# Jingliang-Duan/DSAC-v2

Hardware: NVIDIA H100
Metric: DSAC-T gradient-steps/sec @ batch 4096 (Humanoid-dim) (higher is better)
Workload: dtype bf16x3

## Files before the change

### dsac-v2_b200/_lib.py

```python
from __future__ import annotations

import ctypes as C
import os

_HERE = os.path.dirname(os.path.abspath(__file__))
LIB_PATH = os.environ.get("DSACT_LIB") or os.path.join(_HERE, "libdsact.so")

ABI_VERSION = 4
MAX_HIDDEN = 6
NUM_STATS = 16

ACTIVATIONS = {"linear": 0, "relu": 1, "gelu": 2, "tanh": 3, "sigmoid": 4, "elu": 5, "selu": 6}
GEMM_MODES = {"fp32": 0, "bf16x3": 1, "bf16": 2}
ACT_DISTS = {"TanhGaussDistribution": 0, "GaussDistribution": 1}
POLICY_STDS = {"mlp_shared": 0, "mlp_separated": 1, "parameter": 2}

STATE_STDSUM = 4
STATE_ACC = 16
STATE_STATS = 48


class Config(C.Structure):
    _fields_ = [
        ("abi_version", C.c_int32), ("obs_dim", C.c_int32), ("act_dim", C.c_int32),
# ... 110 lines not shown
    "dsact_seed": (C.c_int, [C.c_void_p, C.c_uint64]),
    "dsact_set_carry": (C.c_int, [C.c_void_p, C.c_float, C.c_float, C.c_int64, C.c_int64, C.c_void_p]),
    "dsact_step": (C.c_int, [C.c_void_p, C.POINTER(Batch), C.POINTER(Noise), C.c_int64, C.c_void_p]),
    "dsact_step_host": (C.c_int, [C.c_void_p, C.POINTER(Batch), C.POINTER(Noise), C.c_int64, C.c_void_p]),
    "dsact_stage_host": (C.c_int, [C.c_void_p, C.POINTER(Batch), C.POINTER(Batch), C.c_void_p]),
    "dsact_stage_release": (C.c_int, [C.c_void_p, C.c_void_p]),
    "dsact_grad_phase1": (C.c_int, [C.c_void_p, C.POINTER(Batch), C.POINTER(Noise), C.c_void_p]),
    "dsact_grad_phase2": (C.c_int, [C.c_void_p, C.c_int64, C.c_void_p]),
    "dsact_compute_grads": (C.c_int, [C.c_void_p, C.POINTER(Batch), C.POINTER(Noise), C.c_void_p]),
    "dsact_apply": (C.c_int, [C.c_void_p, C.c_int64, C.c_void_p]),
    "dsact_read_stats": (C.c_int, [C.c_void_p, C.c_int64, C.c_void_p, C.c_void_p]),
    "dsact_replay_bind": (C.c_int, [C.c_void_p, C.POINTER(Replay)]),
    "dsact_replay_add": (C.c_int, [C.c_void_p] + [C.c_void_p] * 6 + [C.c_int64, C.c_int64, C.c_void_p]),
    "dsact_replay_sample": (C.c_int, [C.c_void_p, C.c_int32, C.c_int64, C.c_void_p, C.POINTER(Batch), C.c_void_p]),
    "dsact_replay_step": (C.c_int, [C.c_void_p, C.c_int32, C.c_int64, C.c_void_p, C.POINTER(Noise), C.c_int64, C.c_void_p]),
    "dsact_replay_steps": (C.c_int, [C.c_void_p, C.c_int32, C.c_int32, C.c_int64, C.c_void_p, C.POINTER(Noise), C.c_void_p,
                                     C.c_int64, C.c_void_p]),
    "dsact_dp_export": (C.c_int, [C.c_void_p, C.c_void_p, C.POINTER(C.c_int64)]),
    "dsact_dp_connect": (C.c_int, [C.c_void_p, C.c_int32, C.c_int32, C.c_void_p]),
    "dsact_dp_step": (C.c_int, [C.c_void_p, C.POINTER(Batch), C.POINTER(Noise), C.c_int64, C.c_int64, C.c_void_p]),
    "dsact_dp_replay_step": (C.c_int, [C.c_void_p, C.c_int32, C.c_int64, C.c_void_p, C.POINTER(Noise), C.c_int64, C.c_int64,
                                       C.c_void_p]),
    "dsact_v1_query_layout": (C.c_int, [C.POINTER(Config), C.POINTER(V1Options), C.POINTER(Layout)]),
    "dsact_v1_create": (C.c_int, [C.POINTER(Config), C.POINTER(V1Options), C.c_int, C.POINTER(C.c_void_p)]),
    "dsact_cnn_query_layout": (C.c_int, [C.POINTER(CnnConfig), C.POINTER(Layout)]),
    "dsact_cnn_create": (C.c_int, [C.POINTER(CnnConfig), C.c_int, C.POINTER(C.c_void_p)]),
    "dsact_profile_step": (C.c_int, [C.c_void_p, C.POINTER(Batch), C.POINTER(Noise), C.c_int64, C.c_void_p, C.POINTER(Profile)]),
    "dsact_launch_count": (C.c_int64, [C.c_void_p]),
    "dsact_last_call_launches": (C.c_int32, [C.c_void_p]),
    "dsact_cnn_test_conv": (C.c_int, [C.c_int32] * 8 + [C.c_void_p] * 7 + [C.c_int32] * 4 + [C.c_void_p]),
    "dsact_test_gemm": (C.c_int, [C.c_void_p, C.c_int32, C.POINTER(TestLayer), C.c_int32, C.c_int32, C.c_void_p]),
    "dsact_test_chain": (C.c_int, [C.c_void_p, C.c_int32, C.c_int32, C.POINTER(C.c_int32), C.c_int32, C.c_int32, C.c_int32,
                                   C.c_int32, C.c_void_p, C.POINTER(TestChainPass), C.c_int32, C.c_void_p]),
    "dsact_test_rows": (C.c_int, [C.c_void_p, C.POINTER(TestRowIo), C.c_void_p]),
    "dsact_test_apply": (C.c_int, [C.c_void_p, C.c_int32, C.c_int32, C.c_int32, C.c_int32, C.c_int64, C.c_int32, C.c_void_p]),
    "dsact_test_dp_attach": (C.c_int, [C.c_void_p, C.c_int32, C.c_int32, C.POINTER(C.c_void_p), C.POINTER(C.c_void_p),
                                       C.POINTER(C.c_int64)]),
    "dsact_test_dp": (C.c_int, [C.c_void_p, C.c_int32, C.POINTER(TestDpIo), C.c_void_p]),
}

_lib = None


class DsactError(RuntimeError):
    pass


def load() -> C.CDLL:
    global _lib
    if _lib is not None:
        return _lib
    if not os.path.exists(LIB_PATH):
        raise DsactError(
            f"{LIB_PATH} is missing: build it with `python -c 'import __graft_entry__ as g; g.build()'` "
            "(nvcc, sm_90a). There is no CPU fallback for the DSAC-T update path.")
    lib = C.CDLL(LIB_PATH)
    for name, (res, args) in SYMBOLS.items():
        fn = getattr(lib, name)
        fn.restype = res
        fn.argtypes = args
    if lib.dsact_abi_version() != ABI_VERSION:
        raise DsactError(f"libdsact.so ABI {lib.dsact_abi_version()} != binding ABI {ABI_VERSION}")
    _lib = lib
    return lib


# ... 4 lines not shown
```

### dsac-v2_b200/csrc/engine.cu

```cuda
#include <cuda_runtime.h>
#include <stdarg.h>
#include <stdio.h>
#include <stdlib.h>
#include <string.h>

#include <algorithm>
#include <cmath>

#include <vector>

#include "../../include/dsact.h"
#include "gemm_simt.cuh"
#include "kernels.cuh"
#include "tc_host.cuh"
#include "chain_tc.cuh"
#include "wgrad_tc.cuh"
#include "dp_peer.cuh"

using namespace dsact;

static thread_local char g_err[512] = "";
static int fail(int code, const char* fmt, ...) {
  va_list ap;
  va_start(ap, fmt);
  vsnprintf(g_err, sizeof(g_err), fmt, ap);
  va_end(ap);
  return code;
}
#define CUDA_TRY(x)                                                                       \
  do {                                                                                    \
    cudaError_t e_ = (x);                                                                 \
    if (e_ != cudaSuccess) return fail(DSACT_ECUDA, "%s failed: %s", #x, cudaGetErrorString(e_)); \
  } while (0)

struct Net {
  int L;
  int s[DSACT_MAX_HIDDEN + 2];
  int64_t w[DSACT_MAX_HIDDEN + 1], b[DSACT_MAX_HIDDEN + 1], n;
  void build(int in, const int32_t* hidden, int L_, int out) {
    L = L_;
    s[0] = in;
    for (int j = 0; j < L; ++j) s[j + 1] = hidden[j];
    s[L + 1] = out;
    n = 0;
    for (int j = 0; j <= L; ++j) {
      w[j] = n; n += (int64_t)s[j + 1] * s[j];
      b[j] = n; n += s[j + 1];
    }
// ... 543 lines not shown
      int blocks = (int)((total + 255) / 256);
      if (blocks < 1) blocks = 1;
      if (blocks > 2 * h->num_sms) blocks = 2 * h->num_sms;
      grid += blocks;
    }
    if (pro) {
      pro->img_blocks = grid;
      launch_k(step_prologue_kernel, grid + pro->zero_blocks + pro->noise_blocks, 256, 0, c, g, *pro);
    } else {
      launch_k(image_kernel, grid, 256, 0, c, g);
    }
    c.done();
    g.n = 0;
  }
};

static ImgOut img_out(const MlpHandle* h, const ImgSlot& s) {
  ImgOut o;
  o.p = nullptr; o.pitch = 0; o.planes = h->passes() == 3 ? 2 : 1; o.plane = 0;
  if (h->tc() && s.off >= 0) { o.p = reinterpret_cast<__nv_bfloat16*>(h->W() + s.off); o.pitch = s.pitch; o.plane = s.plane; }
  return o;
}
static ImgOut img_out_of(const MlpHandle* h, const Img& i) {
  ImgOut o;
  o.p = i.p; o.pitch = i.p ? i.pitch : 0; o.planes = h->passes() == 3 ? 2 : 1; o.plane = i.p ? i.plane : 0;
  return o;
}


struct ChainBuild {
  ChainGroup g;
  int grid = 0, stage_b = 16 * 128;
  int b_mn = -1;
  double flops = 0.0;
  bool ok = true;
  explicit ChainBuild(int passes) { memset(&g, 0, sizeof(g)); g.passes = passes; }
  ChainPass& begin(const Img& a0, const Img& a1, int M) {
    ChainPass& P = g.p[g.n++];
    P.n_layers = 0; P.M = M; P.tile_start = grid;
    grid += (M + TC_BM - 1) / TC_BM;
    ok = ok && make_map(&P.mapA[0], a0, TC_BM);
    if (a1.p) ok = ok && make_map(&P.mapA[1], a1, TC_BM);
    return P;
  }
  ChainLayer& layer(ChainPass& P, const Img& wimg, bool b_mn, int N, int K0, int K1, int kB1) {
    ChainLayer& L = P.L[P.n_layers++];
    L.N = N; L.ldc = N; L.bn = (N + 15) / 16 * 16;
    const int o = b_mn ? 1 : 0;
    if (this->b_mn >= 0 && this->b_mn != o) ok = false;
    this->b_mn = o;
    L.kblocks[0] = (K0 + TC_BK - 1) / TC_BK; L.kblocks[1] = (K1 + TC_BK - 1) / TC_BK;
    L.kB0[0] = 0; L.kB0[1] = kB1;
    ok = ok && make_map(&L.mapB, wimg, b_mn ? 64 : L.bn);
    const int sb = (L.bn + 63) / 64 * 8192;
    if (sb > stage_b) stage_b = sb;
    flops += 2.0 * P.M * N * ((double)K0 + K1);
    return L;
  }
  void image(ChainLayer& L, Img im) {
    if (!im.p) return;
    im.width = (L.N + 7) / 8 * 8;
    L.img = 1;
    ok = ok && make_map(&L.mapImg, im, TC_BM);
  }
};

static void launch_chain(MlpHandle* h, ChainBuild& cb, int cls, Ctx& c) {
  if (cb.g.n == 0) return;
  for (int i = 0; i < cb.g.n; ++i)
    for (int j = 0; j < cb.g.p[i].n_layers; ++j)
      if (cb.g.p[i].L[j].ldc != cb.g.p[i].L[j].N && cb.g.p[i].L[j].Zout) cb.ok = false;
  if (!cb.ok) { c.err = cudaErrorInvalidValue; return; }
  static unsigned long long* dbg = nullptr;
  const bool debug = getenv("DSACT_TC_DEBUG") != nullptr;
  if (debug && !dbg) cudaMalloc(&dbg, sizeof(unsigned long long) * TC_DBG_SLOTS * 4096);
  if (debug && cb.grid <= 4096) { cudaMemsetAsync(dbg, 0, sizeof(unsigned long long) * TC_DBG_SLOTS * cb.grid, c.s); cb.g.dbg = dbg; }
  const int planes = cb.g.passes == 3 ? 2 : 1;
  const int stages = planes == 2 ? 2 : 4;
  const int smem = chain_smem_bytes(stages, planes, cb.stage_b);
  if (!h->chain_attr_done) {
    cudaFuncSetAttribute(tc_chain_kernel<true, false>, cudaFuncAttributeMaxDynamicSharedMemorySize, 227 * 1024);
    cudaFuncSetAttribute(tc_chain_kernel<true, true>, cudaFuncAttributeMaxDynamicSharedMemorySize, 227 * 1024);
    cudaFuncSetAttribute(tc_chain_kernel<false, false>, cudaFuncAttributeMaxDynamicSharedMemorySize, 227 * 1024);
    cudaFuncSetAttribute(tc_chain_kernel<false, true>, cudaFuncAttributeMaxDynamicSharedMemorySize, 227 * 1024);
    h->chain_attr_done = true;
  }
  if (planes == 2) {
    if (cb.b_mn) launch_k(tc_chain_kernel<true, true>, cb.grid, CH_THREADS, smem, c, cb.g, stages, cb.stage_b);
    else launch_k(tc_chain_kernel<true, false>, cb.grid, CH_THREADS, smem, c, cb.g, stages, cb.stage_b);
  } else {
    if (cb.b_mn) launch_k(tc_chain_kernel<false, true>, cb.grid, CH_THREADS, smem, c, cb.g, stages, cb.stage_b);
    else launch_k(tc_chain_kernel<false, false>, cb.grid, CH_THREADS, smem, c, cb.g, stages, cb.stage_b);
  }
  c.done(cls, cb.flops);
  c.check();
  if (debug && cb.g.dbg) {
    cudaStreamSynchronize(c.s);
    std::vector<unsigned long long> hbuf(TC_DBG_SLOTS * (size_t)cb.grid);
    cudaMemcpy(hbuf.data(), dbg, sizeof(unsigned long long) * TC_DBG_SLOTS * cb.grid, cudaMemcpyDeviceToHost);
    unsigned long long tmin = ~0ull, tmax = 0;
    for (int i = 0; i < cb.grid; ++i) {
      const unsigned long long* d = &hbuf[TC_DBG_SLOTS * (size_t)i];
      if (d[0] < tmin) tmin = d[0];
      if (d[6] > tmax) tmax = d[6];
    }
    fprintf(stderr, "[chain_debug] class %d passes %d grid %d span %.1f us\n", cls, cb.g.n, cb.grid, (tmax - tmin) / 1000.0);
    for (int pi = 0; pi < cb.g.n; ++pi) {
      const unsigned long long* d = &hbuf[TC_DBG_SLOTS * (size_t)cb.g.p[pi].tile_start];
      fprintf(stderr, "  pass %d: setup %.1f first-load %.1f |", pi, (d[1] - d[0]) / 1e3, (d[2] - d[0]) / 1e3);
      for (int j = 0; j < cb.g.p[pi].n_layers; ++j)
        fprintf(stderr, " L%d mma-done %.1f epilogue %.1f operand %.1f |", j, (d[8 + 3 * j] - d[0]) / 1e3, (d[9 + 3 * j] - d[0]) / 1e3,
                (d[10 + 3 * j] - d[0]) / 1e3);
      fprintf(stderr, " end %.1f\n", (d[6] - d[0]) / 1e3);
    }
  }
}

struct ChainIo {
  Img w[DSACT_MAX_HIDDEN + 1];
  float* z[DSACT_MAX_HIDDEN] = {};
  Img img[DSACT_MAX_HIDDEN];
  float* colsum[DSACT_MAX_HIDDEN] = {};
};

static ChainPass& chain_fwd_layers(ChainBuild& cb, const Net& net, const float* Wbase, const ChainIo& io, const Img& in0, int k0,
                                   const Img& in1, int k1, int kB1, int B, int act, float* out, int out_ld = 0) {
  ChainPass& P = cb.begin(in0, in1, B);
  for (int j = 0; j <= net.L; ++j) {
    ChainLayer& L = j == 0 ? cb.layer(P, io.w[0], false, net.s[1], k0, k1, kB1) : cb.layer(P, io.w[j], false, net.s[j + 1], net.s[j], 0, 0);
    const bool last = j == net.L;
    L.epi = last ? EPI_STORE : EPI_BIAS_ACT;
    L.act = act;
    L.bias = Wbase + net.b[j];
    if (last) { L.C = out; if (out_ld) L.ldc = out_ld; }
    else {
      L.Zout = io.z[j];
      cb.image(L, io.img[j]);
    }
  }
  return P;
}

static ChainPass& chain_dgrad_layers(ChainBuild& cb, const Net& net, const ChainIo& io, const Img& dout, int B, int act,
                                     float* dact_out, int act_col_img, int act_cols) {
  const Img none;
  ChainPass& P = cb.begin(dout, none, B);
// ... 1634 lines not shown
        x.b = mem.img(t.K0, t.N);
        ibt.add(t.B, t.ldb, x.b, t.K0, t.N);
      }
      if (t.img) {
        x.out.p = static_cast<__nv_bfloat16*>(t.img); x.out.rows = t.M; x.out.width = t.N;
        x.out.pitch = t.img_pitch; x.out.plane = t.img_plane;
      }
      G.wg_off[i] = slab_floats;
      if (variant == V_WGRAD) slab_floats += ((long long)t.M * t.N + 3) / 4 * 4;
    }
    G.push(p, x);
  }
  const int nslabs = 4;
  if (tc) {
    ibt.launch(h, c);
    if (variant == V_WGRAD) {
      G.wg_slab = static_cast<float*>(mem.get(sizeof(float) * (size_t)nslabs * slab_floats));
      G.wg_stride = slab_floats; G.wg_nslabs = nslabs;
      if (G.wg_slab) c.err = cudaMemsetAsync(G.wg_slab, 0xff, sizeof(float) * (size_t)nslabs * slab_floats, c.s);
    }
  }
  if (mem.err == cudaSuccess) launch_group(h, G, variant, c, max_ctas);
  if (tc && variant == V_WGRAD && c.err == cudaSuccess && mem.err == cudaSuccess) {
    for (int i = 0; i < n; ++i) {
      grad_reduce_kernel<<<64, 256, 0, c.s>>>(probs[i].C, G.wg_slab + G.wg_off[i], (long long)probs[i].M * probs[i].N, nslabs,
                                               G.wg_stride);
      c.done();
    }
    c.check();
  }
  return finish_hook(h, c, mem);
}

int dsact_test_chain(dsact_handle* hh, int32_t dgrad, int32_t L, const int32_t* sizes, int32_t K0, int32_t K1, int32_t kB1,
                     int32_t act, const float* params, const dsact_test_chain_pass* passes, int32_t n_passes, void* stream) {
  if (!hh) return fail(DSACT_EINVAL, "null handle");
  int rc = check_mlp(hh, "dsact_test_chain");
  if (rc) return rc;
  MlpHandle* h = mlp(hh);
  if (!h->tc()) return fail(DSACT_EINVAL, "dsact_test_chain: the layer-chain kernel runs in the tensor-core modes only");
  if (!sizes || !params || !passes || L < 0 || L > DSACT_MAX_HIDDEN || n_passes < 1 || n_passes > CH_MAX_PASSES ||
      act < 0 || act > ACT_SELU || (dgrad != 0 && dgrad != 1) || (dgrad && L < 1))
    return fail(DSACT_EINVAL, "bad argument");
  for (int j = 0; j <= L + 1; ++j)
    if (sizes[j] < 1 || (j > 0 && sizes[j] > 256) || (j > 0 && j <= L && sizes[j] % 8))
      return fail(DSACT_EINVAL, "sizes[%d] = %d: widths are >= 1, layer outputs <= 256, hidden widths multiples of 8", j, sizes[j]);
  if (K0 < 1 || K1 < 0 || K0 + K1 != sizes[0] || (K1 > 0 && (kB1 < K0 || kB1 % 8)))
    return fail(DSACT_EINVAL, "layer-0 segments: K0 + K1 == sizes[0], kB1 >= K0, kB1 %% 8 == 0");
  for (int i = 0; i < n_passes; ++i) {
    const dsact_test_chain_pass& q = passes[i];
    if (q.M < 1 || !q.x0 || (!dgrad && (!q.out || (K1 > 0 && !q.x1))) || (dgrad && q.out && K1 == 0) ||
        (q.out_ld != 0 && (dgrad || q.out_ld < sizes[L + 1])))
      return fail(DSACT_EINVAL, "pass %d: bad argument", i);
    for (int j = 0; j < L && dgrad; ++j)
      if (!q.Zin[j]) return fail(DSACT_EINVAL, "pass %d: Zin[%d] is null", i, j);
  }
  CUDA_TRY(cudaSetDevice(h->device));
  Ctx c{(cudaStream_t)stream, 0, cudaSuccess};
  HookScratch mem;
  ImgBatch ibt;
  Net net;
  net.build(sizes[0], sizes + 1, L, sizes[L + 1]);
  ChainIo io;
  for (int j = 0; j <= L; ++j) {
    io.w[j] = mem.img(sizes[j + 1], j == 0 && K1 > 0 ? kB1 + K1 : sizes[j]);
    ibt.reserve(h, c, 1);
    if (j == 0) ibt.add(params + net.w[0], sizes[0], io.w[0], sizes[1], K0, K1, kB1);
    else ibt.add(params + net.w[j], sizes[j], io.w[j], sizes[j + 1], sizes[j]);
  }
  ChainBuild cb(h->passes());
  for (int i = 0; i < n_passes; ++i) {
    const dsact_test_chain_pass& q = passes[i];
    ChainIo pio = io;
    for (int j = 0; j < L; ++j) {
      pio.z[j] = dgrad ? const_cast<float*>(q.Zin[j]) : q.Zout[j];
      pio.colsum[j] = dgrad ? q.colsum[j] : nullptr;
      if (q.img[j]) {
        Img& o = pio.img[j];
        o.p = static_cast<__nv_bfloat16*>(q.img[j]); o.rows = q.M; o.width = sizes[j + 1];
        o.pitch = (sizes[j + 1] + 7) / 8 * 8; o.plane = (long long)o.pitch * q.M;
      }
    }
    const int w0 = dgrad ? sizes[L + 1] : K0;
    ibt.reserve(h, c, 2);
    const Img in0 = mem.img(q.M, w0);
    ibt.add(q.x0, w0, in0, q.M, w0);
    if (dgrad) {
      chain_dgrad_layers(cb, net, pio, in0, q.M, act, q.out, kB1, K1);
    } else {
      Img in1;
      if (K1 > 0) { in1 = mem.img(q.M, K1); ibt.add(q.x1, K1, in1, q.M, K1); }
      chain_fwd_layers(cb, net, params, pio, in0, K0, in1, K1, kB1, q.M, act, q.out, q.out_ld);
    }
  }
  if (mem.err == cudaSuccess) {
    ibt.launch(h, c);
    launch_chain(h, cb, dgrad ? CLS_GEMM_DGRAD : CLS_GEMM_FWD, c);
  }
  return finish_hook(h, c, mem);
}

static int sync_hook(dsact_handle* h, Ctx& c) {
  const cudaError_t e = cudaStreamSynchronize(c.s);
  const cudaError_t err = c.err != cudaSuccess ? c.err : e;
  if (err != cudaSuccess) return fail(DSACT_ECUDA, "launch failed: %s", cudaGetErrorString(err));
  h->launches += c.launches;
  return DSACT_OK;
}

int dsact_test_rows(dsact_handle* h, const dsact_test_row_io* t, void* stream) {
  if (!h || !h->bound) return fail(DSACT_ESTATE, "not bound");
  if (!t) return fail(DSACT_EINVAL, "null rows");
  if (t->kernel < DSACT_TEST_SAMPLE || t->kernel > DSACT_TEST_STATS) return fail(DSACT_EINVAL, "unknown kernel %d", t->kernel);
  const int B = t->batch;
  if (t->kernel != DSACT_TEST_STATS && (B < 1 || B > h->max_batch)) return fail(DSACT_EINVAL, "batch %d outside [1, max_batch]", B);
  if (t->global_batch < (t->kernel == DSACT_TEST_STATS ? 1 : B)) return fail(DSACT_EINVAL, "global_batch < batch");
  if (t->max_blocks < 0) return fail(DSACT_EINVAL, "max_blocks < 0");
  const bool v1 = h->v1, mlp_eng = h->engine == ENGINE_MLP;
  const bool tc = mlp_eng && mlp(h)->tc();
  const int A = h->act_dim, nq = v1 ? 1 : 2;
  const void* imgs[8] = {t->img_act[0], t->img_act[1], t->img_q[0], t->img_q[1], t->img_qa[0], t->img_qa[1], t->img_dlogits,
                         t->img_dlogits_ls};
  for (const void* p : imgs)
    if (p && !tc) return fail(DSACT_EINVAL, "images need a tensor-core mode of the MLP engine");
  auto need = [&](const void* p, const char* what) { return p ? DSACT_OK : fail(DSACT_EINVAL, "%s is null", what); };
  int rc = DSACT_OK;
  RowIo io;
  memset(&io, 0, sizeof(io));
  auto img = [&](void* p, int width) {
    if (!p) return NO_IMG;
    ImgOut o;
    o.p = static_cast<__nv_bfloat16*>(p); o.pitch = (width + 7) / 8 * 8; o.planes = mlp(h)->passes() == 3 ? 2 : 1;
// ... 168 lines not shown
```

### dsac-v2_b200/engine.py

```python
from __future__ import annotations

import ctypes as C
from typing import Dict, Optional, Sequence

import torch

from . import _lib
from ._lib import Batch, Buffers, Config, Layout, Noise, Replay, V1Options, check

STAT_KEYS = [
    "DSAC2/critic_avg_q1-RL iter",
    "DSAC2/critic_avg_q2-RL iter",
    "DSAC2/critic_avg_std1-RL iter",
    "DSAC2/critic_avg_std2-RL iter",
    "DSAC2/critic_avg_min_std1-RL iter",
    "DSAC2/critic_avg_min_std2-RL iter",
    "Loss/Actor loss-RL iter",
    "Loss/Critic loss-RL iter",
    "DSAC2/policy_mean-RL iter",
    "DSAC2/policy_std-RL iter",
    "DSAC2/entropy-RL iter",
    "DSAC2/alpha-RL iter",
    "DSAC2/mean_std1",
    "DSAC2/mean_std2",
# ... 451 lines not shown
        out = {"log_alpha": host[n].clone()}
        for key, tkey, off, cnt, shape in schema:
            out[key] = host[off:off + cnt].view(shape).clone()
            if not grads:
                out[tkey] = thost[off:off + cnt].view(shape).clone()
        return out

    def launch_count(self) -> int:
        return int(self.lib.dsact_launch_count(self.h))

    def last_call_launches(self) -> int:
        return int(self.lib.dsact_last_call_launches(self.h))

    def test_gemm(self, variant: int, A: torch.Tensor, B: torch.Tensor, bias: Optional[torch.Tensor], C_out: torch.Tensor,
                  M: int, N: int, K: int):
        self.test_layers(variant, [dict(M=M, N=N, K0=K, A0=A, B=B, bias=bias, C=C_out)])

    def test_layers(self, variant: int, probs, max_ctas: int = 0):
        arr = (_lib.TestLayer * len(probs))()
        for t, p in zip(arr, probs):
            for k, v in p.items():
                if k == "img":
                    t.img, t.img_pitch, t.img_plane = v.data_ptr(), v.stride(1), v.stride(0)
                elif isinstance(v, torch.Tensor):
                    setattr(t, k, v.data_ptr())
                    ld = {"A0": "lda0", "A1": "lda1", "B": "ldb", "Zin": "ldz", "C": "ldc"}.get(k)
                    if ld and ld not in p:
                        setattr(t, ld, v.stride(0))
                elif v is not None:
                    setattr(t, k, v)
        with torch.cuda.device(self.device):
            check(self.lib.dsact_test_gemm(self.h, variant, arr, len(probs), max_ctas, self._stream()))

    def test_chain(self, dgrad: bool, sizes, K0: int, K1: int, kB1: int, act: int, params: torch.Tensor, passes):
        arr = (_lib.TestChainPass * len(passes))()
        for t, p in zip(arr, passes):
            t.M = p["M"]
            for k in ("x0", "x1", "out"):
                setattr(t, k, _ptr(p.get(k)))
            t.out_ld = int(p.get("out_ld", 0))
            for k in ("Zout", "Zin", "img", "colsum"):
                for j, v in enumerate(p.get(k) or []):
                    getattr(t, k)[j] = _ptr(v)
        sz = (C.c_int32 * len(sizes))(*sizes)
        with torch.cuda.device(self.device):
            check(self.lib.dsact_test_chain(self.h, int(dgrad), len(sizes) - 2, sz, K0, K1, kB1, act, params.data_ptr(), arr,
                                            len(passes), self._stream()))

    def test_rows(self, kernel: str, batch: int, global_batch: Optional[int] = None, max_blocks: int = 0,
                  advance_rng: bool = False, **arrays):
        t = _lib.TestRowIo()
        t.kernel, t.batch = _lib.TEST_KERNELS[kernel], int(batch)
        t.global_batch = int(batch if global_batch is None else global_batch)
        t.max_blocks, t.advance_rng = int(max_blocks), int(bool(advance_rng))
        for k, v in arrays.items():
            if isinstance(v, (list, tuple)):
                for i, x in enumerate(v):
                    getattr(t, k)[i] = _ptr(x)
            else:
                setattr(t, k, v if isinstance(v, int) else _ptr(v))
        with torch.cuda.device(self.device):
            check(self.lib.dsact_test_rows(self.h, C.byref(t), self._stream()))

    def test_apply(self, part: int = 0, fold_slabs: int = 0, scalars_ready: int = 0, tail_rows: int = 0,
                   global_batch: int = 1, max_blocks: int = 0):
        with torch.cuda.device(self.device):
            check(self.lib.dsact_test_apply(self.h, int(part), int(fold_slabs), int(scalars_ready), int(tail_rows),
                                            int(global_batch), int(max_blocks), self._stream()))

    def test_dp_attach(self, rank: int, peers: Sequence["Engine"]) -> torch.Tensor:
        arr = (C.c_void_p * len(peers))(*(p.h.value for p in peers))
        buf, n = C.c_void_p(), C.c_int64()
        with torch.cuda.device(self.device):
            check(self.lib.dsact_test_dp_attach(self.h, int(rank), len(peers), arr, C.byref(buf), C.byref(n)))
        self.dp_world = len(peers)
        self._dp_peers = list(peers)
        return _device_view(buf.value, int(n.value), self.device)

    def test_dp(self, op: str, kind: int = 0, grads: Optional[torch.Tensor] = None, slabs: Optional[torch.Tensor] = None,
                nslabs: int = 0, slab_stride: int = 0, n: int = 0, tail_rows: int = 0, global_batch: int = 1):
# ... 15 lines not shown
```

### include/dsact.h

```cpp
#ifndef DSACT_H
#define DSACT_H

#include <stdint.h>

#ifdef __cplusplus
extern "C" {
#endif

#define DSACT_ABI_VERSION 4
#define DSACT_MAX_HIDDEN 6
#define DSACT_NUM_STATS 16

enum {
  DSACT_OK = 0,
  DSACT_EINVAL = -1,
  DSACT_ECUDA = -2,
  DSACT_ESTATE = -3,
  DSACT_EARCH = -4
};

enum {
  DSACT_ACT_LINEAR = 0, DSACT_ACT_RELU = 1, DSACT_ACT_GELU = 2, DSACT_ACT_TANH = 3,
  DSACT_ACT_SIGMOID = 4, DSACT_ACT_ELU = 5, DSACT_ACT_SELU = 6
};
// ... 156 lines not shown
int dsact_profile_step(dsact_handle *h, const dsact_batch *batch, const dsact_noise *noise, int64_t iteration,
                       void *stream, dsact_profile *out);

typedef struct dsact_test_layer {
  int32_t M, N, K0, K1, kB1;
  const float *A0, *A1, *B;
  int32_t lda0, lda1, ldb;
  int32_t epi, act;
  const float *bias;
  float *Zout;
  const float *Zin;
  int32_t ldz;
  float *colsum;
  float *C;
  int32_t ldc;
  void *img;
  int32_t img_pitch;
  int64_t img_plane;
} dsact_test_layer;
int dsact_test_gemm(dsact_handle *h, int32_t variant, const dsact_test_layer *probs, int32_t n, int32_t max_ctas, void *stream);

typedef struct dsact_test_chain_pass {
  int32_t M;
  const float *x0, *x1;
  float *Zout[DSACT_MAX_HIDDEN];
  const float *Zin[DSACT_MAX_HIDDEN];
  void *img[DSACT_MAX_HIDDEN];
  float *colsum[DSACT_MAX_HIDDEN];
  float *out;
  int32_t out_ld;
} dsact_test_chain_pass;
int dsact_test_chain(dsact_handle *h, int32_t dgrad, int32_t L, const int32_t *sizes, int32_t K0, int32_t K1, int32_t kB1,
                     int32_t act, const float *params, const dsact_test_chain_pass *passes, int32_t n_passes, void *stream);

enum { DSACT_TEST_SAMPLE = 0, DSACT_TEST_LOSS = 1, DSACT_TEST_POLICY_GRAD = 2, DSACT_TEST_STATS = 3 };
typedef struct dsact_test_row_io {
  int32_t kernel, batch;
  int64_t global_batch;
  int32_t max_blocks, advance_rng;
  const float *logits[2], *eps[2];
  float *act[2], *logp[2];
  const float *rew, *done, *z3, *z4;
  const float *out_q[6];
  float *d_out_q[2], *d_out_qa[2];
  const float *d_act[2];
  float *d_logits;
  float *gbias_q[2], *gbias_q_raw[2], *gbias_pi, *gbias_ls;
  void *img_act[2], *img_q[2], *img_qa[2], *img_dlogits;
  float *stats_out;
  void *img_dlogits_ls;
  int32_t split_dlogits;
} dsact_test_row_io;
int dsact_test_rows(dsact_handle *h, const dsact_test_row_io *rows, void *stream);

int dsact_test_apply(dsact_handle *h, int32_t part, int32_t fold_slabs, int32_t scalars_ready, int32_t tail_rows,
                     int64_t global_batch, int32_t max_blocks, void *stream);

int dsact_test_dp_attach(dsact_handle *h, int32_t rank, int32_t world, dsact_handle *const *peers, void **buffer,
                         int64_t *floats);
enum { DSACT_TEST_DP_EXCHANGE = 0, DSACT_TEST_DP_FOLD = 1, DSACT_TEST_DP_REDUCE_SCATTER = 2, DSACT_TEST_DP_APPLY = 3 };
typedef struct dsact_test_dp_io {
  int32_t kind;
  dsact_handle *const *ranks;
  const float *grads, *slabs;
  int32_t nslabs;
  int64_t slab_stride, n;
// ... 21 lines not shown
```

Measured before the change: 2305.

## Add ping-pong two-warpgroup chain kernel selected when grid exceeds one wave

Adds a new fused MLP-chain kernel where each CTA owns two row tiles processed by two consumer warpgroups that alternate tensor-core use through named barriers. One warpgroup's epilogue overlaps the other's WGMMA mainloop, and the weight tiles are split into 128-column halves. The launcher picks this ping-pong variant automatically when the column-split grid would exceed one wave of resident CTAs. The price is a more complex synchronisation scheme, re-created tensor maps, and two half-width B loads per k-block for layers wider than 128.

```diff
diff --git a/dsac-v2_b200/_lib.py b/dsac-v2_b200/_lib.py
--- a/dsac-v2_b200/_lib.py
+++ b/dsac-v2_b200/_lib.py
@@ -166,6 +166,9 @@
     "dsact_test_gemm": (C.c_int, [C.c_void_p, C.c_int32, C.POINTER(TestLayer), C.c_int32, C.c_int32, C.c_void_p]),
     "dsact_test_chain": (C.c_int, [C.c_void_p, C.c_int32, C.c_int32, C.POINTER(C.c_int32), C.c_int32, C.c_int32, C.c_int32,
                                    C.c_int32, C.c_void_p, C.POINTER(TestChainPass), C.c_int32, C.c_void_p]),
+    "dsact_test_chain_tiling": (C.c_int, [C.c_void_p, C.c_int32, C.c_int32, C.c_int32, C.POINTER(C.c_int32), C.c_int32,
+                                          C.c_int32, C.c_int32, C.c_int32, C.c_void_p, C.POINTER(TestChainPass), C.c_int32,
+                                          C.c_void_p]),
     "dsact_test_rows": (C.c_int, [C.c_void_p, C.POINTER(TestRowIo), C.c_void_p]),
     "dsact_test_apply": (C.c_int, [C.c_void_p, C.c_int32, C.c_int32, C.c_int32, C.c_int32, C.c_int64, C.c_int32, C.c_void_p]),
     "dsact_test_dp_attach": (C.c_int, [C.c_void_p, C.c_int32, C.c_int32, C.POINTER(C.c_void_p), C.POINTER(C.c_void_p),
diff --git a/dsac-v2_b200/csrc/chain_pp.cuh b/dsac-v2_b200/csrc/chain_pp.cuh
--- /dev/null
+++ b/dsac-v2_b200/csrc/chain_pp.cuh
@@ -0,0 +1,299 @@
+#pragma once
+#include "chain_tc.cuh"
+
+namespace dsact {
+
+constexpr int PP_HALF = 128;
+constexpr int PP_STAGE_B = PP_HALF * 128;
+constexpr int PP_THREADS = CH_THREADS;
+
+inline int pp_smem_bytes(int stages, int planes) {
+  return stages * planes * PP_STAGE_B + 2 * planes * CH_OPND_PLANE + CH_SCRATCH + 2 * stages * 8 + 1024;
+}
+
+__device__ __forceinline__ uint32_t pp_tid() {
+  uint32_t t;
+  asm volatile("mov.u32 %0, %%tid.x;" : "=r"(t));
+  return t;
+}
+__device__ __forceinline__ int pp_wg() { return (int)(pp_tid() / TC_MMA_THREADS); }
+__device__ __forceinline__ bool pp_lead() { return (pp_tid() & (TC_MMA_THREADS - 1)) == 0; }
+__device__ __forceinline__ void pp_bar() { asm volatile("bar.sync %0, %1;" ::"r"(2 + pp_wg()), "n"(TC_MMA_THREADS) : "memory"); }
+__device__ __forceinline__ void pp_wait_turn() {
+  asm volatile("bar.sync %0, %1;" ::"r"(4 + pp_wg()), "n"(2 * TC_MMA_THREADS) : "memory");
+}
+__device__ __forceinline__ void pp_give_turn() {
+  asm volatile("bar.arrive %0, %1;" ::"r"(5 - pp_wg()), "n"(2 * TC_MMA_THREADS) : "memory");
+}
+
+template <int TB>
+__device__ __forceinline__ void wgmma_n64_hi(float (&d)[128], uint64_t a, uint64_t b) {
+  asm volatile(
+      "{\n\t.reg .pred p;\n\tsetp.ne.b32 p, 1, 0;\n\t"
+      "wgmma.mma_async.sync.aligned.m64n64k16.f32.bf16.bf16 {%0, %1, %2, %3, %4, %5, %6, %7, %8, %9, %10, %11, %12, %13, %14, %15, %16, %17, %18, %19, %20, %21, %22, %23, %24, %25, %26, %27, %28, %29, %30, %31}, %32, %33, p, 1, 1, 0, %34;\n\t}"
+      : "+f"(d[64]), "+f"(d[65]), "+f"(d[66]), "+f"(d[67]), "+f"(d[68]), "+f"(d[69]), "+f"(d[70]), "+f"(d[71]), "+f"(d[72]), "+f"(d[73]), "+f"(d[74]), "+f"(d[75]), "+f"(d[76]), "+f"(d[77]), "+f"(d[78]), "+f"(d[79]), "+f"(d[80]), "+f"(d[81]), "+f"(d[82]), "+f"(d[83]), "+f"(d[84]), "+f"(d[85]), "+f"(d[86]), "+f"(d[87]), "+f"(d[88]), "+f"(d[89]), "+f"(d[90]), "+f"(d[91]), "+f"(d[92]), "+f"(d[93]), "+f"(d[94]), "+f"(d[95])
+      : "l"(a), "l"(b), "n"(TB));
+}
+
+template <int TB>
+__device__ __forceinline__ void wgmma_n128_hi(float (&d)[128], uint64_t a, uint64_t b) {
+  asm volatile(
+      "{\n\t.reg .pred p;\n\tsetp.ne.b32 p, 1, 0;\n\t"
+      "wgmma.mma_async.sync.aligned.m64n128k16.f32.bf16.bf16 {%0, %1, %2, %3, %4, %5, %6, %7, %8, %9, %10, %11, %12, %13, %14, %15, %16, %17, %18, %19, %20, %21, %22, %23, %24, %25, %26, %27, %28, %29, %30, %31, %32, %33, %34, %35, %36, %37, %38, %39, %40, %41, %42, %43, %44, %45, %46, %47, %48, %49, %50, %51, %52, %53, %54, %55, %56, %57, %58, %59, %60, %61, %62, %63}, %64, %65, p, 1, 1, 0, %66;\n\t}"
+      : "+f"(d[64]), "+f"(d[65]), "+f"(d[66]), "+f"(d[67]), "+f"(d[68]), "+f"(d[69]), "+f"(d[70]), "+f"(d[71]), "+f"(d[72]), "+f"(d[73]), "+f"(d[74]), "+f"(d[75]), "+f"(d[76]), "+f"(d[77]), "+f"(d[78]), "+f"(d[79]), "+f"(d[80]), "+f"(d[81]), "+f"(d[82]), "+f"(d[83]), "+f"(d[84]), "+f"(d[85]), "+f"(d[86]), "+f"(d[87]), "+f"(d[88]), "+f"(d[89]), "+f"(d[90]), "+f"(d[91]), "+f"(d[92]), "+f"(d[93]), "+f"(d[94]), "+f"(d[95]), "+f"(d[96]), "+f"(d[97]), "+f"(d[98]), "+f"(d[99]), "+f"(d[100]), "+f"(d[101]), "+f"(d[102]), "+f"(d[103]), "+f"(d[104]), "+f"(d[105]), "+f"(d[106]), "+f"(d[107]), "+f"(d[108]), "+f"(d[109]), "+f"(d[110]), "+f"(d[111]), "+f"(d[112]), "+f"(d[113]), "+f"(d[114]), "+f"(d[115]), "+f"(d[116]), "+f"(d[117]), "+f"(d[118]), "+f"(d[119]), "+f"(d[120]), "+f"(d[121]), "+f"(d[122]), "+f"(d[123]), "+f"(d[124]), "+f"(d[125]), "+f"(d[126]), "+f"(d[127])
+      : "l"(a), "l"(b), "n"(TB));
+}
+
+template <int NBH, int TB, bool PLANES2>
+__device__ __forceinline__ void pp_step_hi(float (&d)[128], uint64_t a_hi, uint64_t b_hi, uint64_t a_lo, uint64_t b_lo) {
+  if constexpr (NBH == 1) {
+    wgmma_n64_hi<TB>(d, a_hi, b_hi);
+    if constexpr (PLANES2) { wgmma_n64_hi<TB>(d, a_hi, b_lo); wgmma_n64_hi<TB>(d, a_lo, b_hi); }
+  } else {
+    wgmma_n128_hi<TB>(d, a_hi, b_hi);
+    if constexpr (PLANES2) { wgmma_n128_hi<TB>(d, a_hi, b_lo); wgmma_n128_hi<TB>(d, a_lo, b_hi); }
+  }
+}
+
+__shared__ int pp_dbg_tile[2];
+#define PP_STAMP(slot) do { if (g.dbg) g.dbg[(size_t)pp_dbg_tile[pp_wg()] * TC_DBG_SLOTS + (slot)] = gtime(); } while (0)
+
+template <bool PLANES2, bool B_MN, int NB>
+__device__ __forceinline__ void pp_layer(const ChainGroup& g, const ChainPass& P, int j, uint8_t* ringB,
+                                         uint8_t* opnd, float* row, int stages, uint64_t* full, uint64_t* empty, int m0,
+                                         int pos, bool wait_turn, bool give_turn) {
+  constexpr int planes = PLANES2 ? 2 : 1;
+  constexpr int NH = NB > 2 ? 2 : 1;
+  constexpr int NB0 = NB > 2 ? 2 : NB;
+  const ChainLayer& Lj = P.L[j];
+  const int lane = threadIdx.x & 31;
+  const int nkb = Lj.kblocks[0] + Lj.kblocks[1];
+  EpiArgs E;
+  E.epi = Lj.epi; E.act = Lj.act; E.M = P.M; E.N = Lj.N; E.ldc = Lj.ldc; E.ldz = Lj.N;
+  E.bias = Lj.bias; E.Zout = Lj.Zout; E.Zin = Lj.Zin; E.colsum = Lj.colsum; E.C = Lj.C;
+  E.img = nullptr;
+  float acc[128];
+#pragma unroll
+  for (int i = 0; i < 32 * NB; ++i) acc[i] = 0.f;
+  int stage = pos % stages, prev = -1;
+  uint32_t phase = (uint32_t)(pos / stages) & 1u;
+  if (wait_turn) pp_wait_turn();
+  for (int kb = 0; kb < nkb; ++kb) {
+    const uint32_t sA = smem_u32(opnd) + (uint32_t)(j == 0 ? (kb & 3) * planes * TC_STAGE_A : kb * TC_STAGE_A);
+    const uint32_t a_plane = j == 0 ? TC_STAGE_A : CH_OPND_PLANE;
+#pragma unroll
+    for (int h = 0; h < NH; ++h) {
+      if (stages == 2 && prev >= 0 && !__all_sync(0xffffffffu, mbar_test(&full[stage], phase))) {
+        wg_wait<0>();
+        if (lane == 0) mbar_arrive(&empty[prev]);
+        prev = -1;
+      }
+      mbar_wait(&full[stage], phase);
+      if (j == 0 && kb == 0 && h == 0 && pp_lead()) PP_STAMP(2);
+      const uint32_t sB = smem_u32(ringB + (size_t)stage * planes * PP_STAGE_B);
+      wg_fence();
+#pragma unroll
+      for (int k = 0; k < TC_BK / 16; ++k) {
+        const uint32_t b_off = B_MN ? k * 2048 : k * 32;
+        const uint64_t b_hi = make_desc(sB + b_off, B_MN ? 8192 : 16, 1024);
+        const uint64_t b_lo = make_desc(sB + PP_STAGE_B + b_off, B_MN ? 8192 : 16, 1024);
+        const uint64_t a_hi = make_desc(sA + k * 32, 16, 1024);
+        const uint64_t a_lo = make_desc(sA + a_plane + k * 32, 16, 1024);
+        if (h == 0) wgmma_step<NB0, 0, B_MN, PLANES2>(acc, a_hi, b_hi, a_lo, b_lo);
+        else pp_step_hi<NB - 2, B_MN, PLANES2>(acc, a_hi, b_hi, a_lo, b_lo);
+      }
+      wg_commit();
+      wg_wait<1>();
+      if (prev >= 0 && lane == 0) mbar_arrive(&empty[prev]);
+      prev = stage;
+      if (++stage == stages) { stage = 0; phase ^= 1; }
+    }
+  }
+  if (give_turn) pp_give_turn();
+  const bool add_bias = (E.epi == EPI_STORE || E.epi == EPI_BIAS_ACT) && E.bias;
+  EpiArgs Eg = E;
+  Eg.bias = nullptr;
+  float one[16];
+#pragma unroll
+  for (int t = 0; t < 16; ++t) one[t] = 1.f;
+  float nx[16];
+  epi_in(nx, E, m0, 0, 0);
+  wg_wait<0>();
+  if (prev >= 0 && lane == 0) mbar_arrive(&empty[prev]);
+  if (pp_lead()) PP_STAMP(8 + 3 * j);
+  const bool opw = j + 1 < P.n_layers || Lj.img;
+  if (opw) {
+    if (pp_lead()) bulk_wait_read();
+    pp_bar();
+  }
+  const int m_row = ((threadIdx.x & (TC_MMA_THREADS - 1)) >> 5) * 16 + ((lane >> 3) & 1) * 8 + (lane & 7);
+  const uint32_t s_row = smem_u32(opnd) + (uint32_t)(m_row * 128);
+#pragma unroll 1
+  for (int q = 0; q < 2 * NB; ++q) {
+    float v[16];
+#pragma unroll
+    for (int c = 0; c < 2 * NB; ++c)
+      if (q == c) {
+#pragma unroll
+        for (int t = 0; t < 16; ++t) v[t] = acc[16 * c + t];
+      }
+    if (add_bias) {
+#pragma unroll
+      for (int t = 0; t < 16; ++t) v[t] += nx[2 * (t >> 2) + (t & 1)];
+    } else if (E.epi == EPI_DACT) {
+#pragma unroll
+      for (int t = 0; t < 16; ++t) v[t] *= nx[t];
+    }
+    if (q + 1 < 2 * NB) epi_in(nx, E, m0, 0, q + 1);
+    epi_group<PLANES2>(v, one, Eg, m0, 0, q, row);
+    if (opw) {
+      uint32_t whi[8], wlo[8];
+#pragma unroll
+      for (int i = 0; i < 8; ++i) {
+        if (PLANES2) split_pack2(v[2 * i], v[2 * i + 1], whi[i], wlo[i]);
+        else whi[i] = cvt_bf16x2(v[2 * i], v[2 * i + 1]);
+      }
+      const uint32_t s_q = s_row + (uint32_t)((q >> 1) * TC_STAGE_A);
+#pragma unroll
+      for (int s = 0; s < 2; ++s) {
+        const uint32_t a = s_q + (uint32_t)((((4 * (q & 1) + 2 * s + (lane >> 4)) ^ (lane & 7))) << 4);
+        stsm_x4(a, whi[4 * s], whi[4 * s + 1], whi[4 * s + 2], whi[4 * s + 3]);
+        if (PLANES2) stsm_x4(a + CH_OPND_PLANE, wlo[4 * s], wlo[4 * s + 1], wlo[4 * s + 2], wlo[4 * s + 3]);
+      }
+    }
+  }
+  if (pp_lead()) PP_STAMP(9 + 3 * j);
+  if (opw) {
+    fence_async_smem();
+    pp_bar();
+    if (Lj.img && pp_lead()) {
+      for (int kb = 0; kb < (Lj.N + 63) / 64; ++kb)
+        for (int pl = 0; pl < planes; ++pl) tma_store_3d(&Lj.mapImg, opnd + pl * CH_OPND_PLANE + kb * TC_STAGE_A, kb * TC_BK, m0, pl);
+      bulk_commit();
+    }
+  }
+  if (pp_lead()) PP_STAMP(10 + 3 * j);
+}
+
+__device__ __forceinline__ int pp_items(const ChainLayer& L) { return (L.kblocks[0] + L.kblocks[1]) * (L.bn > PP_HALF ? 2 : 1); }
+
+template <bool PLANES2, bool B_MN>
+__global__ void __launch_bounds__(PP_THREADS, 1) tc_pingpong_kernel(const __grid_constant__ ChainGroup g, int stages) {
+  extern __shared__ __align__(1024) uint8_t smem_raw[];
+  uint8_t* smem = smem_raw + ((1024u - (smem_u32(smem_raw) & 1023u)) & 1023u);
+  constexpr int planes = PLANES2 ? 2 : 1;
+  uint8_t* ringB = smem;
+  uint8_t* opnd0 = smem + (size_t)stages * planes * PP_STAGE_B;
+  float* scratch = reinterpret_cast<float*>(opnd0 + 2 * planes * CH_OPND_PLANE);
+  uint64_t* bars = reinterpret_cast<uint64_t*>(reinterpret_cast<uint8_t*>(scratch) + CH_SCRATCH);
+  uint64_t* full = bars;
+  uint64_t* empty = bars + stages;
+
+  constexpr int PRODUCER = CH_MMA_THREADS / 32;
+  const int warp = threadIdx.x >> 5, lane = threadIdx.x & 31;
+
+  int pi = 0, cta0 = 0;
+  for (int i = 0; i + 1 < g.n; ++i) {
+    const int c = (g.p[i].M + 2 * TC_BM - 1) / (2 * TC_BM);
+    if ((int)blockIdx.x < cta0 + c) break;
+    cta0 += c;
+    pi = i + 1;
+  }
+  const ChainPass& P = g.p[pi];
+  const int tile0 = 2 * ((int)blockIdx.x - cta0);
+  const int ntiles = min(2, (P.M + TC_BM - 1) / TC_BM - tile0);
+  const int nl = P.n_layers;
+  const int w = threadIdx.x / TC_MMA_THREADS;
+  if (w < ntiles && (threadIdx.x & (TC_MMA_THREADS - 1)) == 0) {
+    pp_dbg_tile[w] = P.tile_start + tile0 + w;
+    PP_STAMP(0);
+  }
+
+  if (threadIdx.x == 0) {
+    for (int s = 0; s < stages; ++s) { mbar_init(&full[s], 1); mbar_init(&empty[s], TC_MMA_THREADS / 32); }
+    asm volatile("fence.mbarrier_init.release.cluster;" ::: "memory");
+  }
+  if (warp == PRODUCER) {
+    for (int i = lane; i < 2 + 2 * nl; i += 32) {
+      const CUtensorMap* m = nullptr;
+      if (i == 0) m = &P.mapA[0];
+      else if (i == 1) { if (P.L[0].kblocks[1] > 0) m = &P.mapA[1]; }
+      else if (i < 2 + nl) m = &P.L[i - 2].mapB;
+      else if (P.L[i - 2 - nl].img) m = &P.L[i - 2 - nl].mapImg;
+      if (m) asm volatile("prefetch.tensormap [%0];" ::"l"(reinterpret_cast<uint64_t>(m)) : "memory");
+    }
+  }
+  __syncthreads();
+  asm volatile("griddepcontrol.wait;" ::: "memory");
+  asm volatile("griddepcontrol.launch_dependents;" ::: "memory");
+  if (w < ntiles && (threadIdx.x & (TC_MMA_THREADS - 1)) == 0) PP_STAMP(1);
+
+  if (threadIdx.x >= CH_MMA_THREADS) {
+    asm volatile("setmaxnreg.dec.sync.aligned.u32 %0;" ::"n"(CH_PRODUCER_REGS));
+    if (warp == PRODUCER && lane == 0) {
+      int stage = 0;
+      uint32_t phase = 0;
+      for (int j = 0; j < nl; ++j) {
+        const ChainLayer& Lj = P.L[j];
+        const int nkb = Lj.kblocks[0] + Lj.kblocks[1];
+        const int nb = (Lj.bn + 63) / 64, nh = nb > 2 ? 2 : 1;
+        for (int t = 0; t < ntiles; ++t) {
+          const int m0 = (tile0 + t) * TC_BM;
+          uint8_t* opnd = opnd0 + (size_t)t * planes * CH_OPND_PLANE;
+          for (int kb = 0; kb < nkb; ++kb) {
+            const int seg = kb >= Lj.kblocks[0] ? 1 : 0;
+            const int kloc = (seg ? kb - Lj.kblocks[0] : kb) * TC_BK;
+            const int kB = Lj.kB0[seg] + kloc;
+            for (int h = 0; h < nh; ++h) {
+              const int boxes = min(2, nb - 2 * h);
+              const uint32_t b_bytes = B_MN ? (uint32_t)boxes * 8192 : (uint32_t)min(Lj.bn, PP_HALF) * 128;
+              const bool a = j == 0 && h == 0;
+              mbar_wait(&empty[stage], phase ^ 1);
+              mbar_expect_tx(&full[stage], planes * (b_bytes + (a ? (uint32_t)TC_STAGE_A : 0u)));
+              uint8_t* sB = ringB + (size_t)stage * planes * PP_STAGE_B;
+              for (int pl = 0; pl < planes; ++pl) {
+                if (a) tma_load_3d(opnd + (size_t)((kb & 3) * planes + pl) * TC_STAGE_A, &P.mapA[seg], &full[stage], kloc, m0, pl);
+                if (B_MN) {
+                  for (int i = 0; i < boxes; ++i)
+                    tma_load_3d(sB + pl * PP_STAGE_B + i * 8192, &Lj.mapB, &full[stage], 64 * (2 * h + i), kB, pl);
+                } else {
+                  tma_load_3d(sB + pl * PP_STAGE_B, &Lj.mapB, &full[stage], kB, PP_HALF * h, pl);
+                }
+              }
+              if (++stage == stages) { stage = 0; phase ^= 1; }
+            }
+          }
+        }
+      }
+    }
+  } else {
+    asm volatile("setmaxnreg.inc.sync.aligned.u32 %0;" ::"n"(CH_MMA_REGS));
+    if (w < ntiles) {
+      float* row = scratch + threadIdx.x * 16;
+      uint8_t* opnd = opnd0 + (size_t)w * planes * CH_OPND_PLANE;
+      const int m0 = (tile0 + w) * TC_BM;
+      int pos = 0;
+      for (int j = 0; j < nl; ++j) {
+        const int items = pp_items(P.L[j]);
+        const int mine = pos + w * items;
+        const bool wait = ntiles == 2 && (w == 1 || j > 0), give = ntiles == 2 && (w == 0 || j + 1 < nl);
+        switch ((P.L[j].bn + 63) / 64) {
+          case 1: pp_layer<PLANES2, B_MN, 1>(g, P, j, ringB, opnd, row, stages, full, empty, m0, mine, wait, give); break;
+          case 2: pp_layer<PLANES2, B_MN, 2>(g, P, j, ringB, opnd, row, stages, full, empty, m0, mine, wait, give); break;
+          case 3: pp_layer<PLANES2, B_MN, 3>(g, P, j, ringB, opnd, row, stages, full, empty, m0, mine, wait, give); break;
+          default: pp_layer<PLANES2, B_MN, 4>(g, P, j, ringB, opnd, row, stages, full, empty, m0, mine, wait, give); break;
+        }
+        pos += items * ntiles;
+      }
+      if ((threadIdx.x & (TC_MMA_THREADS - 1)) == 0) bulk_wait();
+    }
+  }
+
+  if (lane == 0 && w < ntiles) { if (g.dbg) atomicMax(&g.dbg[(size_t)pp_dbg_tile[w] * TC_DBG_SLOTS + 5], gtime()); }
+  __syncthreads();
+  if (w < ntiles && (threadIdx.x & (TC_MMA_THREADS - 1)) == 0) PP_STAMP(6);
+}
+
+#undef PP_STAMP
+
+}
diff --git a/dsac-v2_b200/csrc/engine.cu b/dsac-v2_b200/csrc/engine.cu
--- a/dsac-v2_b200/csrc/engine.cu
+++ b/dsac-v2_b200/csrc/engine.cu
@@ -13,7 +13,7 @@
 #include "gemm_simt.cuh"
 #include "kernels.cuh"
 #include "tc_host.cuh"
-#include "chain_tc.cuh"
+#include "chain_pp.cuh"
 #include "wgrad_tc.cuh"
 #include "dp_peer.cuh"
 
@@ -623,6 +623,7 @@
   ChainGroup g;
   int grid = 0, stage_b = 16 * 128;
   int b_mn = -1;
+  Img w[CH_MAX_PASSES][CH_MAX_LAYERS];
   double flops = 0.0;
   bool ok = true;
   explicit ChainBuild(int passes) { memset(&g, 0, sizeof(g)); g.passes = passes; }
@@ -643,6 +644,7 @@
     L.kblocks[0] = (K0 + TC_BK - 1) / TC_BK; L.kblocks[1] = (K1 + TC_BK - 1) / TC_BK;
     L.kB0[0] = 0; L.kB0[1] = kB1;
     ok = ok && make_map(&L.mapB, wimg, b_mn ? 64 : L.bn);
+    w[&P - g.p][P.n_layers - 1] = wimg;
     const int sb = (L.bn + 63) / 64 * 8192;
     if (sb > stage_b) stage_b = sb;
     flops += 2.0 * P.M * N * ((double)K0 + K1);
@@ -656,7 +658,9 @@
   }
 };
 
-static void launch_chain(MlpHandle* h, ChainBuild& cb, int cls, Ctx& c) {
+enum { CHAIN_BY_SHAPE = -1, CHAIN_COLUMN_SPLIT = 0, CHAIN_PINGPONG = 1 };
+
+static void launch_chain(MlpHandle* h, ChainBuild& cb, int cls, Ctx& c, int tiling = CHAIN_BY_SHAPE) {
   if (cb.g.n == 0) return;
   for (int i = 0; i < cb.g.n; ++i)
     for (int j = 0; j < cb.g.p[i].n_layers; ++j)
@@ -669,14 +673,38 @@
   const int planes = cb.g.passes == 3 ? 2 : 1;
   const int stages = planes == 2 ? 2 : 4;
   const int smem = chain_smem_bytes(stages, planes, cb.stage_b);
+  const int pp_smem = pp_smem_bytes(stages, planes);
   if (!h->chain_attr_done) {
     cudaFuncSetAttribute(tc_chain_kernel<true, false>, cudaFuncAttributeMaxDynamicSharedMemorySize, 227 * 1024);
     cudaFuncSetAttribute(tc_chain_kernel<true, true>, cudaFuncAttributeMaxDynamicSharedMemorySize, 227 * 1024);
     cudaFuncSetAttribute(tc_chain_kernel<false, false>, cudaFuncAttributeMaxDynamicSharedMemorySize, 227 * 1024);
     cudaFuncSetAttribute(tc_chain_kernel<false, true>, cudaFuncAttributeMaxDynamicSharedMemorySize, 227 * 1024);
+    cudaFuncSetAttribute(tc_pingpong_kernel<true, false>, cudaFuncAttributeMaxDynamicSharedMemorySize, 226 * 1024);
+    cudaFuncSetAttribute(tc_pingpong_kernel<true, true>, cudaFuncAttributeMaxDynamicSharedMemorySize, 226 * 1024);
+    cudaFuncSetAttribute(tc_pingpong_kernel<false, false>, cudaFuncAttributeMaxDynamicSharedMemorySize, 226 * 1024);
+    cudaFuncSetAttribute(tc_pingpong_kernel<false, true>, cudaFuncAttributeMaxDynamicSharedMemorySize, 226 * 1024);
     h->chain_attr_done = true;
   }
-  if (planes == 2) {
+  if (tiling == CHAIN_BY_SHAPE) {
+    int per_sm = 0;
+    const cudaError_t e = cudaOccupancyMaxActiveBlocksPerMultiprocessor(&per_sm, tc_chain_kernel<true, false>, CH_THREADS, smem);
+    if (e != cudaSuccess) { c.err = e; return; }
+    tiling = cb.grid > std::max(per_sm, 1) * h->num_sms ? CHAIN_PINGPONG : CHAIN_COLUMN_SPLIT;
+  }
+  if (tiling == CHAIN_PINGPONG) {
+    for (int i = 0; i < cb.g.n && !cb.b_mn; ++i)
+      for (int j = 0; j < cb.g.p[i].n_layers; ++j)
+        if (cb.g.p[i].L[j].bn > PP_HALF && !make_map(&cb.g.p[i].L[j].mapB, cb.w[i][j], PP_HALF)) { c.err = cudaErrorInvalidValue; return; }
+    int ctas = 0;
+    for (int i = 0; i < cb.g.n; ++i) ctas += (cb.g.p[i].M + 2 * TC_BM - 1) / (2 * TC_BM);
+    if (planes == 2) {
+      if (cb.b_mn) launch_k(tc_pingpong_kernel<true, true>, ctas, PP_THREADS, pp_smem, c, cb.g, stages);
+      else launch_k(tc_pingpong_kernel<true, false>, ctas, PP_THREADS, pp_smem, c, cb.g, stages);
+    } else {
+      if (cb.b_mn) launch_k(tc_pingpong_kernel<false, true>, ctas, PP_THREADS, pp_smem, c, cb.g, stages);
+      else launch_k(tc_pingpong_kernel<false, false>, ctas, PP_THREADS, pp_smem, c, cb.g, stages);
+    }
+  } else if (planes == 2) {
     if (cb.b_mn) launch_k(tc_chain_kernel<true, true>, cb.grid, CH_THREADS, smem, c, cb.g, stages, cb.stage_b);
     else launch_k(tc_chain_kernel<true, false>, cb.grid, CH_THREADS, smem, c, cb.g, stages, cb.stage_b);
   } else {
@@ -695,14 +723,19 @@
       if (d[0] < tmin) tmin = d[0];
       if (d[6] > tmax) tmax = d[6];
     }
-    fprintf(stderr, "[chain_debug] class %d passes %d grid %d span %.1f us\n", cls, cb.g.n, cb.grid, (tmax - tmin) / 1000.0);
+    fprintf(stderr, "[chain_debug] class %d passes %d grid %d span %.1f us %s\n", cls, cb.g.n, cb.grid, (tmax - tmin) / 1000.0,
+            tiling == CHAIN_PINGPONG ? "ping-pong" : "column split");
     for (int pi = 0; pi < cb.g.n; ++pi) {
-      const unsigned long long* d = &hbuf[TC_DBG_SLOTS * (size_t)cb.g.p[pi].tile_start];
-      fprintf(stderr, "  pass %d: setup %.1f first-load %.1f |", pi, (d[1] - d[0]) / 1e3, (d[2] - d[0]) / 1e3);
-      for (int j = 0; j < cb.g.p[pi].n_layers; ++j)
-        fprintf(stderr, " L%d mma-done %.1f epilogue %.1f operand %.1f |", j, (d[8 + 3 * j] - d[0]) / 1e3, (d[9 + 3 * j] - d[0]) / 1e3,
-                (d[10 + 3 * j] - d[0]) / 1e3);
-      fprintf(stderr, " end %.1f\n", (d[6] - d[0]) / 1e3);
+      const int t0 = cb.g.p[pi].tile_start, tend = pi + 1 < cb.g.n ? cb.g.p[pi + 1].tile_start : cb.grid;
+      const unsigned long long* d0 = &hbuf[TC_DBG_SLOTS * (size_t)t0];
+      for (int t = t0; t < (tiling == CHAIN_PINGPONG ? std::min(t0 + 2, tend) : t0 + 1); ++t) {
+        const unsigned long long* d = &hbuf[TC_DBG_SLOTS * (size_t)t];
+        fprintf(stderr, "  pass %d tile %d: setup %.1f first-load %.1f |", pi, t - t0, (d[1] - d0[0]) / 1e3, (d[2] - d0[0]) / 1e3);
+        for (int j = 0; j < cb.g.p[pi].n_layers; ++j)
+          fprintf(stderr, " L%d mma-done %.1f epilogue %.1f operand %.1f |", j, (d[8 + 3 * j] - d0[0]) / 1e3,
+                  (d[9 + 3 * j] - d0[0]) / 1e3, (d[10 + 3 * j] - d0[0]) / 1e3);
+        fprintf(stderr, " end %.1f\n", (d[6] - d0[0]) / 1e3);
+      }
     }
   }
 }
@@ -2403,8 +2436,9 @@
   return finish_hook(h, c, mem);
 }
 
-int dsact_test_chain(dsact_handle* hh, int32_t dgrad, int32_t L, const int32_t* sizes, int32_t K0, int32_t K1, int32_t kB1,
-                     int32_t act, const float* params, const dsact_test_chain_pass* passes, int32_t n_passes, void* stream) {
+static int test_chain(dsact_handle* hh, int tiling, int32_t dgrad, int32_t L, const int32_t* sizes, int32_t K0, int32_t K1,
+                      int32_t kB1, int32_t act, const float* params, const dsact_test_chain_pass* passes, int32_t n_passes,
+                      void* stream) {
   if (!hh) return fail(DSACT_EINVAL, "null handle");
   int rc = check_mlp(hh, "dsact_test_chain");
   if (rc) return rc;
@@ -2466,9 +2500,22 @@
   }
   if (mem.err == cudaSuccess) {
     ibt.launch(h, c);
-    launch_chain(h, cb, dgrad ? CLS_GEMM_DGRAD : CLS_GEMM_FWD, c);
+    launch_chain(h, cb, dgrad ? CLS_GEMM_DGRAD : CLS_GEMM_FWD, c, tiling);
   }
   return finish_hook(h, c, mem);
+}
+
+int dsact_test_chain(dsact_handle* h, int32_t dgrad, int32_t L, const int32_t* sizes, int32_t K0, int32_t K1, int32_t kB1,
+                     int32_t act, const float* params, const dsact_test_chain_pass* passes, int32_t n_passes, void* stream) {
+  return test_chain(h, CHAIN_BY_SHAPE, dgrad, L, sizes, K0, K1, kB1, act, params, passes, n_passes, stream);
+}
+
+int dsact_test_chain_tiling(dsact_handle* h, int32_t tiling, int32_t dgrad, int32_t L, const int32_t* sizes, int32_t K0,
+                            int32_t K1, int32_t kB1, int32_t act, const float* params, const dsact_test_chain_pass* passes,
+                            int32_t n_passes, void* stream) {
+  if (tiling != CHAIN_COLUMN_SPLIT && tiling != CHAIN_PINGPONG)
+    return fail(DSACT_EINVAL, "dsact_test_chain_tiling: tiling %d is neither 0 (column split) nor 1 (ping-pong)", tiling);
+  return test_chain(h, tiling, dgrad, L, sizes, K0, K1, kB1, act, params, passes, n_passes, stream);
 }
 
 static int sync_hook(dsact_handle* h, Ctx& c) {
diff --git a/dsac-v2_b200/engine.py b/dsac-v2_b200/engine.py
--- a/dsac-v2_b200/engine.py
+++ b/dsac-v2_b200/engine.py
@@ -507,7 +507,8 @@
         with torch.cuda.device(self.device):
             check(self.lib.dsact_test_gemm(self.h, variant, arr, len(probs), max_ctas, self._stream()))
 
-    def test_chain(self, dgrad: bool, sizes, K0: int, K1: int, kB1: int, act: int, params: torch.Tensor, passes):
+    def test_chain(self, dgrad: bool, sizes, K0: int, K1: int, kB1: int, act: int, params: torch.Tensor, passes,
+                   tiling: Optional[int] = None):
         arr = (_lib.TestChainPass * len(passes))()
         for t, p in zip(arr, passes):
             t.M = p["M"]
@@ -519,8 +520,12 @@
                     getattr(t, k)[j] = _ptr(v)
         sz = (C.c_int32 * len(sizes))(*sizes)
         with torch.cuda.device(self.device):
-            check(self.lib.dsact_test_chain(self.h, int(dgrad), len(sizes) - 2, sz, K0, K1, kB1, act, params.data_ptr(), arr,
-                                            len(passes), self._stream()))
+            if tiling is None:
+                check(self.lib.dsact_test_chain(self.h, int(dgrad), len(sizes) - 2, sz, K0, K1, kB1, act, params.data_ptr(),
+                                                arr, len(passes), self._stream()))
+            else:
+                check(self.lib.dsact_test_chain_tiling(self.h, int(tiling), int(dgrad), len(sizes) - 2, sz, K0, K1, kB1, act,
+                                                       params.data_ptr(), arr, len(passes), self._stream()))
 
     def test_rows(self, kernel: str, batch: int, global_batch: Optional[int] = None, max_blocks: int = 0,
                   advance_rng: bool = False, **arrays):
diff --git a/include/dsact.h b/include/dsact.h
--- a/include/dsact.h
+++ b/include/dsact.h
@@ -212,6 +212,9 @@
 } dsact_test_chain_pass;
 int dsact_test_chain(dsact_handle *h, int32_t dgrad, int32_t L, const int32_t *sizes, int32_t K0, int32_t K1, int32_t kB1,
                      int32_t act, const float *params, const dsact_test_chain_pass *passes, int32_t n_passes, void *stream);
+int dsact_test_chain_tiling(dsact_handle *h, int32_t tiling, int32_t dgrad, int32_t L, const int32_t *sizes, int32_t K0,
+                            int32_t K1, int32_t kB1, int32_t act, const float *params, const dsact_test_chain_pass *passes,
+                            int32_t n_passes, void *stream);
 
 enum { DSACT_TEST_SAMPLE = 0, DSACT_TEST_LOSS = 1, DSACT_TEST_POLICY_GRAD = 2, DSACT_TEST_STATS = 3 };
 typedef struct dsact_test_row_io {
```

New measurement: 2412 (median of 6 runs). +4.7%, better.
